# sp-uhh/audio-visual-vad

Measured on AMD Instinct MI355X. Metric: AV frame-pairs/sec (fwd+bwd), higher is better.
Workload: dtype f32; 1 GPU; AV_net fused training step (WaveNet-W0 encoder + ResNet-18 trunk + concat + 2xLSTM1024 + FC, masked BCE, backward, RCCL all-reduce, fused Adam): BASELINE configs[3]/[4] per-GPU shard; per_gpu_frame_pairs=1024, global_frame_pairs=1024, sequences_per_gpu=64, parallelism=dp1, reserved_cus=0, reported_block=median

## Files before the change

### audio-visual-vad_amd/avvad/_lib.py

```python
import ctypes as C
import os

import torch

_HERE = os.path.dirname(os.path.abspath(__file__))
LIB_PATH = os.environ.get("AVVAD_LIB") or os.path.join(os.path.dirname(_HERE), "lib", "libavvad_hip.so")

TRUNK_NCONV = 20
ABI_VERSION = 3
SCORE_CHUNK = 4096
MIX_CHUNK = 4096
SPECTRAL_CHUNK = 2048
_ERR = {-1: "AVVAD_EINVAL (bad descriptor / unsupported shape)", -2: "AVVAD_EWORKSPACE (workspace too small)",
        -3: "AVVAD_ELAUNCH (kernel launch failed)"}

FP = C.c_void_p


class AvvadError(RuntimeError):
    pass


class GemmDesc(C.Structure):
    _fields_ = [(n, C.c_int) for n in ("M", "N", "K", "lda", "ldb", "ldc", "transA", "transB", "accumulate",
# ... 36 lines not shown

class StftDesc(C.Structure):
    _fields_ = [("B", C.c_int), ("L", C.c_long), ("n_fft", C.c_int), ("hop", C.c_int), ("T", C.c_int), ("eps", C.c_float)]


class StftStreamDesc(C.Structure):
    _fields_ = [("B", C.c_int), ("L", C.c_int), ("n_fft", C.c_int), ("hop", C.c_int), ("T", C.c_int), ("M", C.c_int),
                ("eps", C.c_float), ("norm_eps", C.c_float)]


class IstftDesc(C.Structure):
    _fields_ = [(n, C.c_int) for n in ("B", "T", "n_fft", "hop", "start", "out_pitch", "mask_mode")]


class IstftStreamDesc(C.Structure):
    _fields_ = [(n, C.c_int) for n in ("B", "T", "n_fft", "hop", "L", "M", "mask_mode")]


class TargetDesc(C.Structure):
    _fields_ = [("B", C.c_int), ("L", C.c_long), ("n_fft", C.c_int), ("hop", C.c_int), ("T", C.c_int), ("center", C.c_int),
                ("eps", C.c_float), ("vad_coef", C.c_double), ("ibm_coef", C.c_double)]


class LipDesc(C.Structure):
    _fields_ = [("B", C.c_int), ("n_max", C.c_int), ("rows", C.c_long), ("T", C.c_int), ("W", C.c_int), ("H", C.c_int),
                ("p", C.c_int), ("q", C.c_int), ("quantize", C.c_int), ("norm_eps", C.c_float)]


class LstmDesc(C.Structure):
    _fields_ = [("B", C.c_int), ("T", C.c_int), ("In", C.c_int), ("H", C.c_int), ("lengths", FP),
                ("save_for_backward", C.c_int)]


SIGNATURES = {
    "avvad_version": (C.c_char_p, []),
    "avvad_abi_version": (C.c_int, []),
    "avvad_set_option": (C.c_int, [C.c_char_p, C.c_int]),
    "avvad_get_option": (C.c_int, [C.c_char_p]),
    "avvad_engine_workspace": (C.c_size_t, []),
    "avvad_gemm_f32": (C.c_int, [FP, FP, FP, FP, C.POINTER(GemmDesc), FP, C.c_size_t, FP]),
    "avvad_wavenet_workspace": (C.c_size_t, [C.POINTER(WavenetDesc)]),
    "avvad_wavenet_fwd": (C.c_int, [FP, C.POINTER(WavenetPtrs), FP, C.POINTER(WavenetDesc), FP, C.c_size_t, FP]),
    "avvad_wavenet_bwd": (C.c_int, [FP, C.POINTER(WavenetPtrs), FP, C.POINTER(WavenetPtrs), FP,
                                    C.POINTER(WavenetDesc), FP, C.c_size_t, FP]),
    "avvad_wavenet_block_fwd": (C.c_int, [FP, FP, FP, FP, FP, FP, C.c_int, C.c_int, C.c_int, FP]),
    "avvad_conv2d_pack_weights": (C.c_int, [FP, FP, FP, C.POINTER(ConvDesc), FP]),
    "avvad_conv2d_fwd": (C.c_int, [FP, FP, FP, C.POINTER(ConvDesc), FP, C.c_size_t, FP]),
    "avvad_conv2d_dgrad": (C.c_int, [FP, FP, FP, C.POINTER(ConvDesc), C.c_int, FP, C.c_size_t, FP]),
    "avvad_conv2d_wgrad": (C.c_int, [FP, FP, FP, C.POINTER(ConvDesc), FP, C.c_size_t, FP]),
    "avvad_conv2d_pack_weights_bf16": (C.c_int, [FP, FP, FP, C.POINTER(ConvDesc), FP]),
    "avvad_conv2d_fwd_bf16": (C.c_int, [FP, FP, FP, C.POINTER(ConvDesc), FP, C.c_size_t, FP]),
    "avvad_conv2d_dgrad_bf16": (C.c_int, [FP, FP, FP, C.POINTER(ConvDesc), C.c_int, FP, C.c_size_t, FP]),
    "avvad_conv2d_wgrad_bf16": (C.c_int, [FP, FP, FP, C.POINTER(ConvDesc), FP, C.c_size_t, FP]),
    "avvad_trunk_workspace": (C.c_size_t, [C.POINTER(TrunkDesc)]),
    "avvad_trunk_activation": (C.c_int, [C.POINTER(TrunkDesc), C.c_int, C.POINTER(C.c_size_t), C.POINTER(C.c_int), C.POINTER(C.c_int),
                                         C.POINTER(C.c_int)]),
    "avvad_trunk_fwd": (C.c_int, [FP, C.POINTER(TrunkParams), FP, C.POINTER(TrunkDesc), FP, C.c_size_t, FP]),
    "avvad_trunk_bwd": (C.c_int, [FP, C.POINTER(TrunkParams), FP, C.POINTER(TrunkGrads), C.POINTER(TrunkDesc), FP,
                                  C.c_size_t, FP]),
    "avvad_lstm_workspace": (C.c_size_t, [C.POINTER(LstmDesc)]),
    "avvad_lstm_layer_fwd": (C.c_int, [FP, FP, FP, FP, FP, FP, C.POINTER(LstmDesc), FP, C.c_size_t, FP]),
    "avvad_lstm_layer_bwd": (C.c_int, [FP, FP, FP, FP, FP, FP, FP, FP, FP, FP, C.POINTER(LstmDesc), FP, C.c_size_t, FP]),
    "avvad_lstm_state_workspace": (C.c_size_t, [C.POINTER(LstmDesc)]),
    "avvad_lstm_layer_fwd_state": (C.c_int, [FP] * 10 + [C.POINTER(LstmDesc), FP, C.c_size_t, FP]),
    "avvad_wavenet_stream_state_bytes": (C.c_size_t, [C.POINTER(WavenetDesc)]),
    "avvad_wavenet_stream_workspace": (C.c_size_t, [C.POINTER(WavenetDesc)]),
    "avvad_wavenet_stream_fwd": (C.c_int, [FP, C.POINTER(WavenetPtrs), FP, FP, FP, C.c_int, FP, C.c_int,
                                           C.POINTER(WavenetDesc), FP, C.c_size_t, FP]),
    "avvad_mcb_workspace": (C.c_size_t, [C.POINTER(McbDesc)]),
    "avvad_mcb_fusion_fwd": (C.c_int, [FP] * 11 + [C.POINTER(McbDesc), FP, C.c_size_t, FP]),
    "avvad_mcb_fusion_bwd": (C.c_int, [FP] * 12 + [C.POINTER(McbDesc), FP, C.c_size_t, FP]),
    "avvad_count_sketch_fwd": (C.c_int, [FP, FP, FP, FP, C.c_int, C.c_int, C.c_int, FP]),
    "avvad_count_sketch_bwd": (C.c_int, [FP, FP, FP, FP, C.c_int, C.c_int, C.c_int, FP]),
    "avvad_mcb_fwd": (C.c_int, [FP] * 7 + [C.c_int] * 4 + [FP]),
    "avvad_mcb_bwd": (C.c_int, [FP] * 9 + [C.c_int] * 4 + [FP]),
    "avvad_stft_workspace": (C.c_size_t, [C.POINTER(StftDesc)]),
    "avvad_stft": (C.c_int, [FP, FP, C.POINTER(StftDesc), C.c_int, FP, C.c_size_t, FP]),
    "avvad_stft_features": (C.c_int, [FP, FP, FP, FP, C.POINTER(StftDesc), C.c_float, FP, C.c_size_t, FP]),
    "avvad_abs_max": (C.c_int, [FP, FP, C.c_int, C.c_long, FP]),
    "avvad_stft_stream_basis_bytes": (C.c_size_t, [C.c_int]),
    "avvad_stft_stream_basis": (C.c_int, [C.c_int, FP, FP]),
    "avvad_stft_stream_fwd": (C.c_int, [FP] * 12 + [C.POINTER(StftStreamDesc), FP]),
    "avvad_stft_stream_fwd_spec": (C.c_int, [FP] * 13 + [C.POINTER(StftStreamDesc), FP]),
    "avvad_istft_stream_basis_bytes": (C.c_size_t, [C.c_int]),
    "avvad_istft_stream_basis": (C.c_int, [C.c_int, FP, FP]),
    "avvad_istft_stream_workspace": (C.c_size_t, [C.POINTER(IstftStreamDesc)]),
    "avvad_istft_stream": (C.c_int, [FP] * 10 + [C.POINTER(IstftStreamDesc), FP, C.c_size_t, FP]),
    "avvad_istft_workspace": (C.c_size_t, [C.POINTER(IstftDesc)]),
    "avvad_istft": (C.c_int, [FP, C.c_long, C.c_long, C.c_long, FP, FP, FP, FP, FP, C.POINTER(IstftDesc), FP, C.c_size_t, FP]),
    "avvad_resynth_workspace": (C.c_size_t, [C.POINTER(StftDesc), C.POINTER(IstftDesc)]),
    "avvad_resynth": (C.c_int, [FP, FP, FP, FP, FP, FP, C.POINTER(StftDesc), C.POINTER(IstftDesc), FP, C.c_size_t, FP]),
    "avvad_istft_bwd_workspace": (C.c_size_t, [C.POINTER(IstftDesc)]),
    "avvad_istft_bwd": (C.c_int, [FP, C.c_long, C.c_long, C.c_long, FP, FP, FP, FP, FP, FP, C.POINTER(IstftDesc), FP, C.c_size_t,
                                  FP]),
    "avvad_resynth_bwd_workspace": (C.c_size_t, [C.POINTER(StftDesc), C.POINTER(IstftDesc)]),
    "avvad_resynth_bwd": (C.c_int, [FP, FP, FP, FP, FP, FP, FP, C.POINTER(StftDesc), C.POINTER(IstftDesc), FP, C.c_size_t, FP]),
    "avvad_stft_complex": (C.c_int, [FP, FP, C.POINTER(StftDesc), FP, C.c_size_t, FP]),
    "avvad_stats_workspace": (C.c_size_t, [C.c_size_t, C.c_int]),
    "avvad_stats_accumulate": (C.c_int, [FP, FP, FP, C.c_int, C.c_int, C.c_int, C.c_int, FP, C.c_size_t, FP]),
    "avvad_stft_stats_workspace": (C.c_size_t, [C.POINTER(StftDesc)]),
    "avvad_stft_stats": (C.c_int, [FP, FP, FP, C.POINTER(StftDesc), FP, C.c_size_t, FP]),
    "avvad_stats_finalize": (C.c_int, [FP, C.c_int, FP, FP, FP]),
    "avvad_score_workspace": (C.c_size_t, [C.c_int, C.c_long]),
    "avvad_score_accumulate": (C.c_int, [FP, C.c_long, FP, C.c_long, FP, C.c_long, C.c_int, FP, FP, C.c_int, C.c_long, FP,
                                         C.c_size_t, FP]),
    "avvad_score_finalize": (C.c_int, [FP, C.c_int, C.c_int, FP, FP, FP]),
# ... 77 lines not shown
```

### audio-visual-vad_amd/csrc/common.h

```cpp
#pragma once
#include <hip/hip_runtime.h>
#include <stdint.h>
#include <atomic>

#include "avvad.h"

typedef float f32x16 __attribute__((ext_vector_type(16)));
typedef float f32x4 __attribute__((ext_vector_type(4)));

#include <stdio.h>
#define AVVAD_LAUNCH_CHECK()                                                                      \
  do {                                                                                            \
    hipError_t e_ = hipGetLastError();                                                            \
    if (e_ != hipSuccess) {                                                                       \
      fprintf(stderr, "avvad: HIP error '%s' after launch at %s:%d\n", hipGetErrorString(e_), __FILE__, __LINE__); \
      return AVVAD_ELAUNCH;                                                                       \
    }                                                                                             \
  } while (0)

#define AVVAD_ENTER() (void)hipGetLastError()

struct AvvadTune {
  int igemm_variant;
  int no_streamk;
  int kmajor;
  int lstm_no_fused_step;
  int lstm_no_persistent;
  int no_stem_kernel;
  int no_tall;
  int wn_no_fused_tail;
  int wn_no_tail_pair;
  int wn_no_fused_wgrad;
  int no_fixup1;
  int no_buf;
  int wn_flat;
  int wn_dx;
  int wn_grid;
  int wn_bwd_t;
  int bf16;
  int stagger;
  int cls_cap;
  int no_cls;
  int no_fused_stats;
  int no_s2_cls;
  int no_conv64;
  int bwd_max_cus;
  int max_cus;
};
AvvadTune& avvad_tune();
struct BwdCuCap {
  int saved;
  BwdCuCap() : saved(avvad_tune().max_cus) {
    const int b = avvad_tune().bwd_max_cus;
    if (b > 0 && (saved <= 0 || b < saved)) avvad_tune().max_cus = b;
  }
  ~BwdCuCap() { avvad_tune().max_cus = saved; }
};
static inline int grid_cus() {
  const int m = avvad_tune().max_cus;
  return (m > 0 && m < 256) ? m : 256;
}

template <auto Kernel>
int allow_large_lds(size_t bytes, size_t limit) {
  if (bytes <= 64 * 1024) return AVVAD_OK;
  static std::atomic<unsigned char> allowed[64];
  int dev = -1;
  if (hipGetDevice(&dev) != hipSuccess) return AVVAD_ELAUNCH;
  const bool known = dev >= 0 && dev < 64;
  if (known && allowed[dev].load(std::memory_order_acquire)) return AVVAD_OK;
  if (hipFuncSetAttribute(reinterpret_cast<const void*>(Kernel), hipFuncAttributeMaxDynamicSharedMemorySize, (int)limit) != hipSuccess)
    return AVVAD_ELAUNCH;
  if (known) allowed[dev].store(1, std::memory_order_release);
  return AVVAD_OK;
}

static inline int cdiv(long a, long b) { return (int)((a + b - 1) / b); }
static inline size_t align_up(size_t v, size_t a) { return (v + a - 1) / a * a; }
static inline bool ws_misaligned(const void* p) { return ((uintptr_t)p & 15) != 0; }
__device__ __forceinline__ int clamp_count(int v, int hi) { return v < 0 ? 0 : (v > hi ? hi : v); }

__device__ __forceinline__ f32x16 mfma32(float a, float b, f32x16 c) {
  return __builtin_amdgcn_mfma_f32_32x32x2f32(a, b, c, 0, 0, 0);
}
__device__ __forceinline__ float relu1(float x) {
  const int v = __builtin_bit_cast(int, x);
  return __builtin_bit_cast(float, v > 0 ? v : 0);
// ... 56 lines not shown
```

### audio-visual-vad_amd/csrc/misc.hip

```cpp
#include "common.h"

extern "C" const char* avvad_version(void) { return "avvad-hip 0.1 (gfx950, fp32 MFMA)"; }
extern "C" int avvad_abi_version(void) { return AVVAD_ABI_VERSION; }

#include <stdlib.h>
#include <string.h>
namespace {
struct OptName { const char* name; const char* env; int AvvadTune::*field; };
const OptName kOpts[] = {
    {"igemm_variant", "AVVAD_IGEMM_VARIANT", &AvvadTune::igemm_variant},
    {"no_streamk", "AVVAD_NO_STREAMK", &AvvadTune::no_streamk},
    {"kmajor", "AVVAD_KMAJOR", &AvvadTune::kmajor},
    {"lstm_no_fused_step", "AVVAD_LSTM_NO_FUSED_STEP", &AvvadTune::lstm_no_fused_step},
    {"lstm_no_persistent", "AVVAD_LSTM_NO_PERSISTENT", &AvvadTune::lstm_no_persistent},
    {"no_stem_kernel", "AVVAD_NO_STEM_KERNEL", &AvvadTune::no_stem_kernel},
    {"no_tall", "AVVAD_NO_TALL", &AvvadTune::no_tall},
    {"wn_no_fused_tail", "AVVAD_WN_NO_FUSED_TAIL", &AvvadTune::wn_no_fused_tail},
    {"wn_no_tail_pair", "AVVAD_WN_NO_TAIL_PAIR", &AvvadTune::wn_no_tail_pair},
    {"wn_no_fused_wgrad", "AVVAD_WN_NO_FUSED_WGRAD", &AvvadTune::wn_no_fused_wgrad},
    {"wn_bwd_t", "AVVAD_WN_BWD_T", &AvvadTune::wn_bwd_t},
    {"no_buf", "AVVAD_NO_BUF", &AvvadTune::no_buf},
    {"no_fixup1", "AVVAD_NO_FIXUP1", &AvvadTune::no_fixup1},
    {"no_conv64", "AVVAD_NO_CONV64", &AvvadTune::no_conv64},
    {"no_s2_cls", "AVVAD_NO_S2_CLS", &AvvadTune::no_s2_cls},
    {"wn_flat", "AVVAD_WN_FLAT", &AvvadTune::wn_flat},
    {"wn_grid", "AVVAD_WN_GRID", &AvvadTune::wn_grid},
    {"wn_dx", "AVVAD_WN_DX", &AvvadTune::wn_dx},
    {"bf16", "AVVAD_BF16", &AvvadTune::bf16},
    {"no_fused_stats", "AVVAD_NO_FUSED_STATS", &AvvadTune::no_fused_stats},
    {"no_cls", "AVVAD_NO_CLS", &AvvadTune::no_cls},
    {"cls_cap", "AVVAD_CLS_CAP", &AvvadTune::cls_cap},
    {"stagger", "AVVAD_STAGGER", &AvvadTune::stagger},
    {"max_cus", "AVVAD_MAX_CUS", &AvvadTune::max_cus},
    {"bwd_max_cus", "AVVAD_BWD_MAX_CUS", &AvvadTune::bwd_max_cus},
};
int parse_opt(const char* name, const char* v) {
  if (!strcmp(name, "igemm_variant")) return v[0] == 'd' ? 0 : (v[0] == 's' ? 1 : (v[0] == 'w' ? 2 : atoi(v)));
  if (!strcmp(name, "no_streamk")) return v[0] == 'a' ? 1 : (v[0] >= '0' && v[0] <= '9' && !v[1] ? 10 + (v[0] - '0') : atoi(v));
  if (!strcmp(name, "max_cus") || !strcmp(name, "bwd_max_cus") || !strcmp(name, "wn_flat") || !strcmp(name, "wn_grid") || !strcmp(name, "wn_dx") || !strcmp(name, "wn_bwd_t") || !strcmp(name, "no_fixup1") || !strcmp(name, "cls_cap")) return atoi(v);
  return (v[0] && strcmp(v, "0")) ? 1 : 0;
}
}

AvvadTune& avvad_tune() {
  static AvvadTune t = [] {
    AvvadTune x;
    memset(&x, 0, sizeof(x));
    x.igemm_variant = -1;
    for (const OptName& o : kOpts) {
      const char* v = getenv(o.env);
      if (v && v[0]) x.*(o.field) = parse_opt(o.name, v);
    }
    return x;
  }();
  return t;
}

extern "C" int avvad_set_option(const char* name, int value) {
  if (!name) return AVVAD_EINVAL;
  for (const OptName& o : kOpts)
    if (!strcmp(o.name, name)) { avvad_tune().*(o.field) = value; return AVVAD_OK; }
  return AVVAD_EINVAL;
}

extern "C" int avvad_get_option(const char* name) {
  if (!name) return AVVAD_EINVAL;
  for (const OptName& o : kOpts)
    if (!strcmp(o.name, name)) return avvad_tune().*(o.field);
  return AVVAD_EINVAL;
}

namespace {

__global__ void __launch_bounds__(1024)
    bce_masked_kernel(const float* __restrict__ logits, const float* __restrict__ targets, const int* __restrict__ lengths,
                      float* __restrict__ loss, float* __restrict__ dlogits, int B, int T, int Y, float eps) {
  __shared__ float sm[1024];
// ... 256 lines not shown
```

### audio-visual-vad_amd/csrc/trunk.hip

```cpp
#include "bgemm.h"
#include "conv64.h"

using convop::Geom;

namespace {

#include "bn_kernels.h"

constexpr int NCONV = AVVAD_TRUNK_NCONV;

constexpr int NBLOCK = 8;
constexpr int WIDTHS[4] = {64, 128, 256, 512};

struct Block {
  int stage, width;
  int h, w;
  long M;
  bool ds;
  int i1, i2, id;
  size_t in;
  size_t c1, a1;
  size_t c2, cd;
  size_t out, qm;
};
// ... 977 lines not shown
extern "C" int avvad_debug_prof_clk(unsigned long long* out, int n) {
  hipMemcpyFromSymbol(out, HIP_SYMBOL(igemm::g_prof_clk), sizeof(unsigned long long) * n);
  return 0;
}
extern "C" int avvad_debug_prof_hw(unsigned long long* out, int n) {
  hipMemcpyFromSymbol(out, HIP_SYMBOL(igemm::g_prof_hw), sizeof(unsigned long long) * n);
  return 0;
}
#endif
extern "C" int avvad_conv2d_dgrad(const float* dy, const float* wd, float* dx, const avvad_conv_desc* d, int accumulate,
                                  void* ws, size_t ws_bytes, avvad_stream_t s) {
  return conv2d_dgrad(false, dy, wd, dx, d, accumulate, ws, ws_bytes, s);
}
extern "C" int avvad_conv2d_wgrad(const float* x, const float* dy, float* dw_packed, const avvad_conv_desc* d, void* ws,
                                  size_t ws_bytes, avvad_stream_t s) {
  return conv2d_wgrad(false, x, dy, dw_packed, d, ws, ws_bytes, s);
}

namespace {
__global__ void pack_weights_bf16(const float* __restrict__ w, __bf16* __restrict__ wf16, __bf16* __restrict__ wd16, int Co, int C, int KS) {
  const int T = KS * KS, n = Co * C * T;
  for (int i = blockIdx.x * blockDim.x + threadIdx.x; i < n; i += gridDim.x * blockDim.x) {
    int r = i;
    const int tap = r % T; r /= T;
    const int c = r % C; const int co = r / C;
    const __bf16 v = (__bf16)w[i];
    wf16[(long)co * (T * C) + ((c >> 6) * T + tap) * 64 + (c & 63)] = v;
    if (wd16) wd16[(long)c * (T * Co) + ((co >> 6) * T + tap) * 64 + (co & 63)] = v;
  }
}
}
extern "C" int avvad_conv2d_pack_weights_bf16(const float* w_oihw, void* wf16, void* wd16, const avvad_conv_desc* d, avvad_stream_t s) {
  AVVAD_ENTER();
  Geom g;
  if (!w_oihw || !wf16 || !conv_geom(d, &g) || g.C % 64 || g.Co % 64) return AVVAD_EINVAL;
  hipLaunchKernelGGL(pack_weights_bf16, dim3(ew_grid((long)g.Co * g.C * g.KS * g.KS)), dim3(256), 0, (hipStream_t)s, w_oihw,
                     (__bf16*)wf16, (__bf16*)wd16, g.Co, g.C, g.KS);
  AVVAD_LAUNCH_CHECK();
  return AVVAD_OK;
}
extern "C" int avvad_conv2d_fwd_bf16(const void* x16, const void* wf16, float* y, const avvad_conv_desc* d, void* ws, size_t ws_bytes,
                                     avvad_stream_t s) {
  return conv2d_fwd(true, x16, wf16, y, d, ws, ws_bytes, s);
}
extern "C" int avvad_conv2d_dgrad_bf16(const void* dy16, const void* wd16, float* dx, const avvad_conv_desc* d, int accumulate,
                                       void* ws, size_t ws_bytes, avvad_stream_t s) {
  return conv2d_dgrad(true, dy16, wd16, dx, d, accumulate, ws, ws_bytes, s);
}
extern "C" int avvad_conv2d_wgrad_bf16(const void* x16, const void* dy16, float* dw_packed, const avvad_conv_desc* d, void* ws,
                                       size_t ws_bytes, avvad_stream_t s) {
  return conv2d_wgrad(true, x16, dy16, dw_packed, d, ws, ws_bytes, s);
}

extern "C" size_t avvad_trunk_workspace(const avvad_trunk_desc* d) {
  if (!trunk_desc_ok(d)) return 0;
  const Plan p = make_plan(d);
  return p.total * sizeof(float);
}

extern "C" int avvad_trunk_activation(const avvad_trunk_desc* d, int index, size_t* offset_floats, int* C, int* H, int* W) {
  constexpr int ARGMAX = 1 + 2 * NBLOCK;
  if (!trunk_desc_ok(d) || index < 0 || index > ARGMAX || !offset_floats || !C || !H || !W) return AVVAD_EINVAL;
  if (index == ARGMAX && !d->save_for_backward) return AVVAD_EINVAL;
  const Plan p = make_plan(d);
  if (index == 0 || index == ARGMAX) {
    *offset_floats = index == 0 ? p.p0 : p.am; *C = 64; *H = p.h[2]; *W = p.w[2];
    return AVVAD_OK;
  }
  const Block& k = p.block[(index - 1) / 2];
  *offset_floats = (index - 1) % 2 == 0 ? k.a1 : k.out;
  *C = k.width; *H = k.h; *W = k.w;
  return AVVAD_OK;
}

extern "C" int avvad_trunk_fwd(const float* frames, const avvad_trunk_params* prm, float* feat, const avvad_trunk_desc* d,
                               void* wsv, size_t ws_bytes, avvad_stream_t sv) {
  AVVAD_ENTER();
  if (!frames || !prm || !feat || !wsv || ws_misaligned(wsv) || !trunk_desc_ok(d)) return AVVAD_EINVAL;
  const Plan p = make_plan(d);
  if (ws_bytes < p.total * sizeof(float)) return AVVAD_EWORKSPACE;
  const Run r{p, (float*)wsv, prm, nullptr, d, (hipStream_t)sv};
  hipStream_t s = r.s; int rc;
  const bool b16 = native_bf16();
  const bool save = d->save_for_backward;
  PackTab tab;
  const int nb = tab_shapes(tab, p, cdiv(64 * 49, 256));
  for (int i = 0; i < NCONV; ++i) {
    tab.w[i] = prm->conv_w[i];
    tab.wf[i] = r.at(p.wf[i]);
    tab.wd[i] = (i > 0 && save) ? r.at(p.wd[i]) : nullptr;
    tab.wf16[i] = (b16 && i > 0) ? reinterpret_cast<__bf16*>(r.at(p.wf16[i])) : nullptr;
    tab.wd16[i] = (b16 && i > 0 && save) ? reinterpret_cast<__bf16*>(r.at(p.wd16[i])) : nullptr;
  }
  hipLaunchKernelGGL(pack_all, dim3(nb), dim3(256), 0, s, tab);
  if ((rc = conv_bn(r, 0, frames, r.at(p.c0)))) return rc;
  const BnSlots bn0 = r.bn(0);
  unsigned* am = save ? reinterpret_cast<unsigned*>(r.at(p.am)) : nullptr;
  auto pool = b16 ? stem_bn_relu_pool<true> : stem_bn_relu_pool<false>;
  hipLaunchKernelGGL(pool, dim3(ew_grid((long)d->N * p.h[2] * p.w[2] * 16)), dim3(256), 0, s, r.at(p.c0), bn0.scale, bn0.shift, r.at(p.p0), am,
                     d->N, p.h[1], p.w[1], p.h[2], p.w[2]);
  auto act = b16 ? bn_act<true, false> : bn_act<false, false>;
  auto act_id = b16 ? bn_act<true, true> : bn_act<false, false>;
  for (const Block& k : p.block) {
    const int C = k.width;
    const long nq = k.M * C / 4;
    const float* x = r.at(k.in);
    unsigned char* qmo = save ? reinterpret_cast<unsigned char*>(r.at(k.qm)) : nullptr;
    const BnSlots bn1 = r.bn(k.i1), bn2 = r.bn(k.i2);
    if ((rc = conv_bn(r, k.i1, x, r.at(k.c1)))) return rc;
    hipLaunchKernelGGL(act, dim3(ew_grid(nq)), dim3(256), 0, s, r.at(k.c1), bn1.scale, bn1.shift, NOF, NOF, NOF, r.at(k.a1), nq, C, 1,
                       (unsigned char*)nullptr);
    if ((rc = conv_bn(r, k.i2, r.at(k.a1), r.at(k.c2)))) return rc;
    if (k.ds) {
      if ((rc = conv_bn(r, k.id, x, r.at(k.cd)))) return rc;
      const BnSlots bnd = r.bn(k.id);
      hipLaunchKernelGGL(act, dim3(ew_grid(nq)), dim3(256), 0, s, r.at(k.c2), bn2.scale, bn2.shift, r.at(k.cd), bnd.scale, bnd.shift,
                         r.at(k.out), nq, C, 1, qmo);
    } else {
      hipLaunchKernelGGL(act_id, dim3(ew_grid(nq)), dim3(256), 0, s, r.at(k.c2), bn2.scale, bn2.shift, x, NOF, NOF, r.at(k.out), nq, C, 1, qmo);
    }
  }
  const Block& last = p.block[NBLOCK - 1];
  auto avg = b16 ? avgpool_fwd<true> : avgpool_fwd<false>;
  hipLaunchKernelGGL(avg, dim3(ew_grid((long)d->N * last.width)), dim3(256), 0, s, r.at(last.out), feat, d->N, last.h * last.w, last.width);
  AVVAD_LAUNCH_CHECK();
  return AVVAD_OK;
}

extern "C" int avvad_trunk_bwd(const float* frames, const avvad_trunk_params* prm, const float* dfeat,
                               const avvad_trunk_grads* g, const avvad_trunk_desc* d, void* wsv, size_t ws_bytes,
                               avvad_stream_t sv) {
  AVVAD_ENTER();
  BwdCuCap cu_cap;
  if (!frames || !prm || !dfeat || !g || !wsv || ws_misaligned(wsv) || !trunk_desc_ok(d) || !d->save_for_backward) return AVVAD_EINVAL;
  const Plan p = make_plan(d);
  if (ws_bytes < p.total * sizeof(float)) return AVVAD_EWORKSPACE;
  const Run r{p, (float*)wsv, prm, g, d, (hipStream_t)sv};
  hipStream_t s = r.s; int rc;
  float *G0 = r.at(p.G[0]), *G1 = r.at(p.G[1]), *G2 = r.at(p.G[2]), *G3 = r.at(p.G[3]);
  const Block& last = p.block[NBLOCK - 1];
  hipLaunchKernelGGL(avgpool_bwd, dim3(ew_grid(last.M * last.width)), dim3(256), 0, s, dfeat, G0, d->N, last.h * last.w, last.width);
  const bool b16 = native_bf16();
  const size_t* wd = b16 ? p.wd16 : p.wd;
  auto wgrad = [&](int i, const float* x, const float* dy) {
    return g->conv_w[i] ? conv_wgrad(i > 0 && b16, x, dy, r.at(p.wg[i]), p.geom[i], s, r.at(p.slab)) : AVVAD_OK;
  };
  auto dgrad = [&](int i, const float* dy, float* dx, int acc) { return conv_dgrad(b16, dy, r.at(wd[i]), dx, p.geom[i], acc, s, r.at(p.slab)); };
  for (int kb = NBLOCK - 1; kb >= 0; --kb) {
    const Block& k = p.block[kb];
    const float* x = r.at(k.in);
    BnBwd under_out, under_own;
    under_out.ymask = r.at(k.out);
    under_out.qmask = reinterpret_cast<const unsigned char*>(r.at(k.qm));
    under_out.out16 = under_own.out16 = b16; under_own.own_relu = true;
    if (k.ds) {
      if ((rc = bn_backward(r, k.i2, r.at(k.c2), G0, G1, under_out))) return rc;
      if ((rc = bn_backward(r, k.id, r.at(k.cd), G0, G2, under_out))) return rc;
      if ((rc = wgrad(k.id, x, G2))) return rc;
      if ((rc = dgrad(k.id, G2, G3, 0))) return rc;
    } else {
      under_out.gout = G3;
      if ((rc = bn_backward(r, k.i2, r.at(k.c2), G0, G1, under_out))) return rc;
    }
    if ((rc = wgrad(k.i2, r.at(k.a1), G1))) return rc;
    if ((rc = dgrad(k.i2, G1, G2, 0))) return rc;
    if ((rc = bn_backward(r, k.i1, r.at(k.c1), G2, G1, under_own))) return rc;
    if ((rc = wgrad(k.i1, x, G1))) return rc;
    if ((rc = dgrad(k.i1, G1, G3, 1))) return rc;
    float* t = G0; G0 = G3; G3 = t;
  }
  if (g->conv_w[0] || g->bn_w[0] || g->bn_b[0]) {
    float* g0 = r.at(p.g0);
    const BnSlots bn0 = r.bn(0);
    const bool fuse0 = !avvad_tune().no_fused_stats;
    int grid0 = ew_grid((long)d->N * p.h[1] * p.w[1] * 16);
    if (fuse0 && grid0 > 2048) grid0 = 2048;
    hipLaunchKernelGGL(stem_pool_relu_bwd, dim3(grid0), dim3(256), 0, s, r.at(p.c0), bn0.scale, bn0.shift,
                       reinterpret_cast<const unsigned*>(r.at(p.am)), G0, g0, d->N, p.h[1], p.w[1], p.h[2], p.w[2],
                       fuse0 ? bn0.mean : NOF, fuse0 ? bn0.invstd : NOF, fuse0 ? r.part() : (double*)nullptr);
    BnBwd stem; stem.reduced_chunks = fuse0 ? grid0 : 0;
    if ((rc = bn_backward(r, 0, r.at(p.c0), g0, g0, stem))) return rc;
    if ((rc = wgrad(0, frames, g0))) return rc;
  }
  UnpackTab tab;
  const int nb = tab_shapes(tab, p, cdiv(64 * 3 * 49, 256));
  bool any = false;
  for (int i = 0; i < NCONV; ++i) {
    tab.pk[i] = r.at(p.wg[i]);
    tab.dw[i] = g->conv_w[i];
    any = any || g->conv_w[i];
  }
  if (any) hipLaunchKernelGGL(unpack_all, dim3(nb), dim3(256), 0, s, tab);
  AVVAD_LAUNCH_CHECK();
  return AVVAD_OK;
}
```

### include/avvad.h

```cpp
#ifndef AVVAD_H
#define AVVAD_H

#include <stddef.h>
#include <stdint.h>

#ifdef __cplusplus
extern "C" {
#endif

typedef void* avvad_stream_t;

#define AVVAD_OK 0
#define AVVAD_EINVAL (-1)
#define AVVAD_EWORKSPACE (-2)
#define AVVAD_ELAUNCH (-3)

#define AVVAD_ABI_VERSION 3
const char* avvad_version(void);
int avvad_abi_version(void);

int avvad_set_option(const char* name, int value);
int avvad_get_option(const char* name);

typedef struct {
// ... 50 lines not shown
size_t avvad_wavenet_workspace(const avvad_wavenet_desc* d);
int avvad_wavenet_fwd(const float* wave, const avvad_wavenet_params* p, float* out,
                      const avvad_wavenet_desc* d, void* ws, size_t ws_bytes, avvad_stream_t s);
int avvad_wavenet_bwd(const float* wave, const avvad_wavenet_params* p, const float* dout,
                      const avvad_wavenet_grads* g, float* dwave, const avvad_wavenet_desc* d,
                      void* ws, size_t ws_bytes, avvad_stream_t s);

int avvad_wavenet_block_fwd(const float* s_in, const float* w_dil, const float* b_dil, const float* w_dense,
                            const float* b_dense, float* s_out, int B, int Lin, int dil, avvad_stream_t s);

#define AVVAD_TRUNK_NCONV 20

typedef struct {
  int N, H, W;
  int training;
  float momentum;
  float eps;
  int save_for_backward;
} avvad_trunk_desc;

typedef struct {
  const float* conv_w[AVVAD_TRUNK_NCONV];
  const float* bn_w[AVVAD_TRUNK_NCONV];
  const float* bn_b[AVVAD_TRUNK_NCONV];
  float* bn_rm[AVVAD_TRUNK_NCONV];
  float* bn_rv[AVVAD_TRUNK_NCONV];
} avvad_trunk_params;

typedef struct {
  float* conv_w[AVVAD_TRUNK_NCONV];
  float* bn_w[AVVAD_TRUNK_NCONV];
  float* bn_b[AVVAD_TRUNK_NCONV];
} avvad_trunk_grads;

typedef struct {
  int N, H, W, C, Co, KS, stride, pad;
} avvad_conv_desc;
int avvad_conv2d_pack_weights(const float* w_oihw, float* wf, float* wd, const avvad_conv_desc* d,
                              avvad_stream_t s);
int avvad_conv2d_fwd(const float* x, const float* wf, float* y, const avvad_conv_desc* d, void* ws,
                     size_t ws_bytes, avvad_stream_t s);
int avvad_conv2d_dgrad(const float* dy, const float* wd, float* dx, const avvad_conv_desc* d,
                       int accumulate, void* ws, size_t ws_bytes, avvad_stream_t s);
int avvad_conv2d_wgrad(const float* x, const float* dy, float* dw_packed, const avvad_conv_desc* d, void* ws,
                       size_t ws_bytes, avvad_stream_t s);

int avvad_conv2d_pack_weights_bf16(const float* w_oihw, void* wf16, void* wd16, const avvad_conv_desc* d, avvad_stream_t s);
int avvad_conv2d_fwd_bf16(const void* x16, const void* wf16, float* y, const avvad_conv_desc* d, void* ws, size_t ws_bytes,
                          avvad_stream_t s);
int avvad_conv2d_dgrad_bf16(const void* dy16, const void* wd16, float* dx, const avvad_conv_desc* d, int accumulate,
                            void* ws, size_t ws_bytes, avvad_stream_t s);
int avvad_conv2d_wgrad_bf16(const void* x16, const void* dy16, float* dw_packed, const avvad_conv_desc* d, void* ws,
                            size_t ws_bytes, avvad_stream_t s);

size_t avvad_trunk_workspace(const avvad_trunk_desc* d);
int avvad_trunk_activation(const avvad_trunk_desc* d, int index, size_t* offset_floats, int* C, int* H, int* W);
int avvad_trunk_fwd(const float* frames, const avvad_trunk_params* p, float* feat ,
                    const avvad_trunk_desc* d, void* ws, size_t ws_bytes, avvad_stream_t s);
int avvad_trunk_bwd(const float* frames, const avvad_trunk_params* p, const float* dfeat,
                    const avvad_trunk_grads* g, const avvad_trunk_desc* d, void* ws, size_t ws_bytes,
                    avvad_stream_t s);

typedef struct {
  int B, T, In, H;
  const int* lengths;
  int save_for_backward;
} avvad_lstm_desc;
size_t avvad_lstm_workspace(const avvad_lstm_desc* d);
int avvad_lstm_layer_fwd(const float* x, const float* w_ih, const float* w_hh, const float* b_ih,
                         const float* b_hh, float* y, const avvad_lstm_desc* d, void* ws,
                         size_t ws_bytes, avvad_stream_t s);
int avvad_lstm_layer_bwd(const float* x, const float* w_ih, const float* w_hh, const float* y,
                         const float* dy, float* dx, float* dw_ih, float* dw_hh, float* db_ih,
                         float* db_hh, const avvad_lstm_desc* d, void* ws, size_t ws_bytes,
                         avvad_stream_t s);

size_t avvad_lstm_state_workspace(const avvad_lstm_desc* d);
int avvad_lstm_layer_fwd_state(const float* x, const float* w_ih, const float* w_hh, const float* b_ih,
                               const float* b_hh, const float* h0, const float* c0, float* y, float* hT, float* cT,
                               const avvad_lstm_desc* d, void* ws, size_t ws_bytes, avvad_stream_t s);

size_t avvad_wavenet_stream_state_bytes(const avvad_wavenet_desc* d);
size_t avvad_wavenet_stream_workspace(const avvad_wavenet_desc* d);
int avvad_wavenet_stream_fwd(const float* chunk, const avvad_wavenet_params* p, float* state, const int* n_valid,
                             const int* skip, int k, float* out, int out_frames, const avvad_wavenet_desc* d, void* ws,
                             size_t ws_bytes, avvad_stream_t s);

typedef struct {
  int rows, A, V, D;
  float eps;
  int training;
  float momentum;
  int save_for_backward;
} avvad_mcb_desc;
size_t avvad_mcb_workspace(const avvad_mcb_desc* d);
int avvad_mcb_fusion_fwd(const float* audio, const float* video, const int64_t* h1, const float* s1,
                         const int64_t* h2, const float* s2, const float* bn_w, const float* bn_b,
                         float* bn_rm, float* bn_rv, float* out, const avvad_mcb_desc* d, void* ws,
                         size_t ws_bytes, avvad_stream_t s);
int avvad_mcb_fusion_bwd(const float* audio, const float* video, const int64_t* h1, const float* s1,
                         const int64_t* h2, const float* s2, const float* bn_w, const float* dout,
                         float* daudio, float* dvideo, float* dbn_w, float* dbn_b,
                         const avvad_mcb_desc* d, void* ws, size_t ws_bytes, avvad_stream_t s);

int avvad_count_sketch_fwd(const float* x, const int64_t* h, const float* s, float* out, int rows, int In, int D,
                           avvad_stream_t st);
// ... 186 lines not shown
```

Baseline: 60860 frame-pairs/s.

## Fuse stride-2 downsample block dgrad with shortcut 1x1 dgrad via parity-decomposed kernel

Adds a specialised data-gradient kernel for the 64->128 stride-2 3x3 conv in the ResNet trunk. It splits the input-gradient pixels into four parity classes and computes each from only the taps that reach it. The shortcut 1x1 stride-2 conv dgrad is folded into the same accumulation, replacing two dgrad launches plus an accumulate pass. A standalone pointwise stride-2 dgrad kernel is also added for other downsample shortcuts; it writes zeros to the pixels the stride skips. Both kernels reuse the stream-K-style split/fixup planning of the existing implicit GEMM. They are limited to f32 and to specific shapes, and fall back to the generic path otherwise.

```diff
diff --git a/audio-visual-vad_amd/avvad/_lib.py b/audio-visual-vad_amd/avvad/_lib.py
--- a/audio-visual-vad_amd/avvad/_lib.py
+++ b/audio-visual-vad_amd/avvad/_lib.py
@@ -112,6 +112,8 @@
     "avvad_conv2d_fwd_bf16": (C.c_int, [FP, FP, FP, C.POINTER(ConvDesc), FP, C.c_size_t, FP]),
     "avvad_conv2d_dgrad_bf16": (C.c_int, [FP, FP, FP, C.POINTER(ConvDesc), C.c_int, FP, C.c_size_t, FP]),
     "avvad_conv2d_wgrad_bf16": (C.c_int, [FP, FP, FP, C.POINTER(ConvDesc), FP, C.c_size_t, FP]),
+    "avvad_entry_dgrad": (C.c_int, [FP, FP, FP, FP, FP, C.POINTER(ConvDesc), FP, C.c_size_t, FP]),
+    "avvad_pointwise_dgrad": (C.c_int, [FP, FP, FP, C.POINTER(ConvDesc), FP, C.c_size_t, FP]),
     "avvad_trunk_workspace": (C.c_size_t, [C.POINTER(TrunkDesc)]),
     "avvad_trunk_activation": (C.c_int, [C.POINTER(TrunkDesc), C.c_int, C.POINTER(C.c_size_t), C.POINTER(C.c_int), C.POINTER(C.c_int),
                                          C.POINTER(C.c_int)]),
diff --git a/audio-visual-vad_amd/csrc/common.h b/audio-visual-vad_amd/csrc/common.h
--- a/audio-visual-vad_amd/csrc/common.h
+++ b/audio-visual-vad_amd/csrc/common.h
@@ -33,6 +33,7 @@
   int wn_no_fused_wgrad;
   int no_fixup1;
   int no_buf;
+  int no_entry;
   int wn_flat;
   int wn_dx;
   int wn_grid;
diff --git a/audio-visual-vad_amd/csrc/entry.h b/audio-visual-vad_amd/csrc/entry.h
--- /dev/null
+++ b/audio-visual-vad_amd/csrc/entry.h
@@ -0,0 +1,282 @@
+#pragma once
+#include "common.h"
+
+namespace entry {
+
+constexpr int NW = 8;
+constexpr int MAXROWS = 512;
+
+struct Prod { int G, base, rt; };
+struct Sched { int w1, w2, w3, w4; int has_ds; Prod ds, c0, c1, c2, c3; };
+
+struct Cut {
+  unsigned R, G, it0, g, nb;
+  bool split;
+  __device__ __forceinline__ void init(int te, const Prod& P, int kt) {
+    split = P.rt > 0 && te >= P.base;
+    if (!split) return;
+    R = (unsigned)P.rt * (unsigned)kt; G = (unsigned)P.G; it0 = (unsigned)(te - P.base) * (unsigned)kt;
+    g = ((it0 + 1u) * G + R - 1u) / R - 1u;
+    nb = (g + 1u) * R / G;
+  }
+  __device__ __forceinline__ bool ends(int j, int kt) {
+    if (j == kt - 1) return true;
+    if (!split || it0 + (unsigned)j + 1u < nb) return false;
+    do { ++g; nb = (g + 1u) * R / G; } while (nb <= it0 + (unsigned)j + 1u);
+    return true;
+  }
+};
+
+#define ENTRY_CONTRACT(av, row0)                                                                                  \
+  do {                                                                                                            \
+    const float* const bt_ = wl + ((row0) + lh) * 64 + li;                                                        \
+    float b_[2][8];                                                                                               \
+    _Pragma("unroll") for (int s_ = 0; s_ < 4; ++s_) { b_[0][2 * s_] = bt_[s_ * 128]; b_[0][2 * s_ + 1] = bt_[s_ * 128 + 32]; } \
+    _Pragma("unroll") for (int j_ = 0; j_ < 4; ++j_) {                                                            \
+      if (j_ < 3) {                                                                                               \
+        _Pragma("unroll") for (int s_ = 0; s_ < 4; ++s_) {                                                        \
+          b_[(j_ + 1) & 1][2 * s_] = bt_[((j_ + 1) * 4 + s_) * 128];                                              \
+          b_[(j_ + 1) & 1][2 * s_ + 1] = bt_[((j_ + 1) * 4 + s_) * 128 + 32];                                     \
+        }                                                                                                         \
+      }                                                                                                           \
+      __builtin_amdgcn_sched_barrier(0);                                                                          \
+      _Pragma("unroll") for (int s_ = 0; s_ < 4; ++s_) {                                                          \
+        const int i_ = j_ * 4 + s_;                                                                               \
+        const float a_ = lh ? av[i_ >> 1][2 * (i_ & 1) + 1] : av[i_ >> 1][2 * (i_ & 1)];                          \
+        acc0 = mfma32(a_, b_[j_ & 1][2 * s_], acc0);                                                              \
+        acc1 = mfma32(a_, b_[j_ & 1][2 * s_ + 1], acc1);                                                          \
+      }                                                                                                           \
+      __builtin_amdgcn_sched_barrier(0);                                                                          \
+    }                                                                                                             \
+  } while (0)
+#define ENTRY_FLUSH(last)                                                                                         \
+  do {                                                                                                            \
+    if (npiece == 0) {                                                                                            \
+      _Pragma("unroll") for (int r_ = 0; r_ < 16; ++r_) { val0[r_] = val0[r_] + (acc0[r_] + 0.f); val1[r_] = val1[r_] + (acc1[r_] + 0.f); } \
+    } else {                                                                                                      \
+      _Pragma("unroll") for (int r_ = 0; r_ < 16; ++r_) { sum0[r_] = sum0[r_] + acc0[r_]; sum1[r_] = sum1[r_] + acc1[r_]; } \
+    }                                                                                                             \
+    ++npiece;                                                                                                     \
+    _Pragma("unroll") for (int r_ = 0; r_ < 16; ++r_) { acc0[r_] = 0.f; acc1[r_] = 0.f; }                         \
+    if (last) {                                                                                                   \
+      if (npiece > 1) {                                                                                           \
+        _Pragma("unroll") for (int r_ = 0; r_ < 16; ++r_) { val0[r_] = val0[r_] + sum0[r_]; val1[r_] = val1[r_] + sum1[r_]; } \
+      }                                                                                                           \
+      _Pragma("unroll") for (int r_ = 0; r_ < 16; ++r_) { sum0[r_] = 0.f; sum1[r_] = 0.f; }                       \
+      npiece = 0;                                                                                                 \
+    }                                                                                                             \
+  } while (0)
+
+__global__ void __launch_bounds__(NW * 64, 2)
+    dgrad_kernel(const float* __restrict__ dy, const float* __restrict__ wd, const float* __restrict__ dd, const float* __restrict__ wdd,
+                 float* __restrict__ dx, const int N, const int H, const int W, const int Ho, const int Wo, const Sched sc) {
+  __shared__ __attribute__((aligned(16))) float wl[MAXROWS * 64];
+  const int t = threadIdx.x, lane = t & 63, wave = t >> 6;
+  const int li = lane & 31, lh = lane >> 5;
+  const int bid = blockIdx.x;
+  const int q = (bid >= sc.w1 ? 1 : 0) + (bid >= sc.w2 ? 1 : 0) + (bid >= sc.w3 ? 1 : 0);
+  const int ph = q >> 1, pw = q & 1;
+  const int b0 = q == 0 ? 0 : (q == 1 ? sc.w1 : (q == 2 ? sc.w2 : sc.w3));
+  const int b1 = q == 0 ? sc.w1 : (q == 1 ? sc.w2 : (q == 2 ? sc.w3 : sc.w4));
+  const Prod pc = q == 0 ? sc.c0 : (q == 1 ? sc.c1 : (q == 2 ? sc.c2 : sc.c3));
+  const int Hc = (H - ph + 1) >> 1, Wc = (W - pw + 1) >> 1, HWc = Hc * Wc, Mc = N * HWc;
+  const unsigned mg_hw = HWc > 1 ? (unsigned)(0x100000000ull / (unsigned)HWc + 1ull) : 0u;
+  const unsigned mg_w = Wc > 1 ? (unsigned)(0x100000000ull / (unsigned)Wc + 1ull) : 0u;
+  const int ntap = (1 + ph) * (1 + pw), tsh = ph + pw;
+  const int nds = (q == 0 && sc.has_ds) ? 4 : 0;
+  const int ktc = 4 * ntap, nstep = nds + ktc;
+  const __amdgpu_buffer_rsrc_t rx = brsrc2g(dy);
+  const __amdgpu_buffer_rsrc_t rd = brsrc2g(sc.has_ds ? dd : dy);
+  const __amdgpu_buffer_rsrc_t ro = brsrc2g(dx);
+  const long T = ((long)Mc + 31) / 32, G = b1 - b0;
+  const long t_lo = (bid - b0) * T / G, t_hi = (bid - b0 + 1) * T / G;
+
+  struct Step { int delta, need, row; bool ds; };
+  auto step = [&](int s) -> Step {
+    if (s < nds) return {s * 128, 0, ntap * 128 + s * 32, true};
+    const int j = s - nds, cc = j >> tsh, tp = j & (ntap - 1);
+    const int ia = pw ? tp >> 1 : tp, ib = pw ? tp & 1 : 0;
+    const int dho = ph ? 1 - ia : 0, dwo = pw ? 1 - ib : 0;
+    return {(dho * Wo + dwo) * 512 + cc * 128, dho | (dwo << 1), tp * 128 + cc * 32, false};
+  };
+  int pixbase = 0, vmask = 0;
+  auto tile_ctx = [&](long tile) {
+    const int m = (int)tile * 32 + li;
+    const int n = mg_hw ? (int)__umulhi((unsigned)m, mg_hw) : m, r = m - n * HWc;
+    const int hc = mg_w ? (int)__umulhi((unsigned)r, mg_w) : r, wc = r - hc * Wc;
+    const int okh = hc + 1 < Ho ? 1 : 0, okw = wc + 1 < Wo ? 1 : 0;
+    vmask = m < Mc ? (1 | (okh << 1) | (okw << 2) | ((okh & okw) << 3)) : 0;
+    pixbase = ((n * Ho + hc) * Wo + wc) * 512;
+  };
+  f4v a0[8], a1[8];
+  f32x16 acc0, acc1, val0, val1, sum0, sum1;
+  auto fetch = [&](f4v (&av)[8], int s) {
+    const Step st = step(s);
+    const int vo = ((vmask >> st.need) & 1) ? pixbase + st.delta : BUF_OOB;
+    if (st.ds) {
+#pragma unroll
+      for (int j = 0; j < 8; ++j) av[j] = bload4(rd, vo + j * 16, 0);
+    } else {
+#pragma unroll
+      for (int j = 0; j < 8; ++j) av[j] = bload4(rx, vo + j * 16, 0);
+    }
+  };
+
+  long tile = t_lo + wave;
+  if (tile < t_hi) {
+    tile_ctx(tile);
+    fetch(a0, 0);
+  }
+  for (int u = 0; u < ntap + (nds ? 1 : 0); ++u) {
+    const int ia = pw ? u >> 1 : u, ib = pw ? u & 1 : 0;
+    const int kh = ph ? 2 * ia : 1, kw = pw ? 2 * ib : 1;
+    const float4* src = reinterpret_cast<const float4*>(u < ntap ? wd + (long)(kh * 3 + kw) * 128 * 64 : wdd);
+    float4* dst = reinterpret_cast<float4*>(wl + u * 128 * 64);
+#pragma unroll
+    for (int i = t; i < 128 * 16; i += NW * 64) dst[i] = src[i];
+  }
+  __syncthreads();
+#pragma unroll
+  for (int r = 0; r < 16; ++r) { acc0[r] = 0.f; acc1[r] = 0.f; sum0[r] = 0.f; sum1[r] = 0.f; }
+  for (; tile < t_hi; tile += NW) {
+#pragma unroll
+    for (int r = 0; r < 16; ++r) { val0[r] = 0.f; val1[r] = 0.f; }
+    const int m0 = (int)tile * 32;
+    const int te = __builtin_amdgcn_readfirstlane(m0 >> 7);
+    Cut cutd, cutc;
+    cutd.split = false;
+    if (nds) cutd.init(te, sc.ds, 4);
+    cutc.init(te, pc, ktc);
+    int npiece = 0;
+    const bool more = tile + NW < t_hi;
+#pragma unroll 1
+    for (int s = 0; s < nstep; s += 2) {
+      fetch(a1, s + 1);
+      ENTRY_CONTRACT(a0, step(s).row);
+      if (s < nds ? cutd.ends(s, 4) : cutc.ends(s - nds, ktc)) ENTRY_FLUSH(s == nds - 1 || s == nstep - 1);
+      if (s + 2 < nstep) {
+        fetch(a0, s + 2);
+      } else if (more) {
+        tile_ctx(tile + NW);
+        fetch(a0, 0);
+      }
+      ENTRY_CONTRACT(a1, step(s + 1).row);
+      if (s + 1 < nds ? cutd.ends(s + 1, 4) : cutc.ends(s + 1 - nds, ktc)) ENTRY_FLUSH(s + 1 == nds - 1 || s + 1 == nstep - 1);
+    }
+#pragma unroll
+    for (int r = 0; r < 16; ++r) {
+      const int m = m0 + mfma32_row(r, lh);
+      const int n = mg_hw ? (int)__umulhi((unsigned)m, mg_hw) : m, rr = m - n * HWc;
+      const int hc = mg_w ? (int)__umulhi((unsigned)rr, mg_w) : rr, wc = rr - hc * Wc;
+      const int vo = m < Mc ? (((n * H + 2 * hc + ph) * W + 2 * wc + pw) * 64 + li) * 4 : BUF_OOB;
+      bstore(val0[r], ro, vo, 0);
+      bstore(val1[r], ro, vo, 128);
+    }
+  }
+}
+
+__global__ void __launch_bounds__(NW * 64, 2)
+    pw_dgrad_kernel(const float* __restrict__ dd, const float* __restrict__ wd, float* __restrict__ dx, const int N, const int H,
+                    const int W, const int Ho, const int Wo, const int C, const int Co, const int ncb, const int bn, const int ntn,
+                    const Prod pp) {
+  __shared__ __attribute__((aligned(16))) float wl[MAXROWS * 64];
+  const int t = threadIdx.x, lane = t & 63, wave = t >> 6;
+  const int li = lane & 31, lh = lane >> 5;
+  const int pg = blockIdx.x / ncb, cb = blockIdx.x - pg * ncb;
+  const int HWo = Ho * Wo, M = N * HWo;
+  const unsigned mg_hw = HWo > 1 ? (unsigned)(0x100000000ull / (unsigned)HWo + 1ull) : 0u;
+  const unsigned mg_w = Wo > 1 ? (unsigned)(0x100000000ull / (unsigned)Wo + 1ull) : 0u;
+  const int kt = Co >> 5;
+  const __amdgpu_buffer_rsrc_t rx = brsrc2g(dd);
+  const __amdgpu_buffer_rsrc_t ro = brsrc2g(dx);
+  const long T = ((long)M + 31) / 32, G = gridDim.x / ncb;
+  const long t_lo = pg * T / G, t_hi = (pg + 1) * T / G;
+  const int pix = Co * 4;
+  f4v a0[8], a1[8];
+  f32x16 acc0, acc1, val0, val1, sum0, sum1;
+  auto fetch = [&](f4v (&av)[8], long tile, int s) {
+    const int m = (int)tile * 32 + li;
+    const int vo = m < M ? m * pix + s * 128 : BUF_OOB;
+#pragma unroll
+    for (int j = 0; j < 8; ++j) av[j] = bload4(rx, vo + j * 16, 0);
+  };
+  long tile = t_lo + wave;
+  if (tile < t_hi) fetch(a0, tile, 0);
+  for (int i = t; i < Co * 16; i += NW * 64)
+    reinterpret_cast<float4*>(wl)[i] = *reinterpret_cast<const float4*>(wd + (long)(i >> 4) * C + cb * 64 + (i & 15) * 4);
+  __syncthreads();
+#pragma unroll
+  for (int r = 0; r < 16; ++r) { acc0[r] = 0.f; acc1[r] = 0.f; sum0[r] = 0.f; sum1[r] = 0.f; }
+  for (; tile < t_hi; tile += NW) {
+#pragma unroll
+    for (int r = 0; r < 16; ++r) { val0[r] = 0.f; val1[r] = 0.f; }
+    const int m0 = (int)tile * 32;
+    const int te = __builtin_amdgcn_readfirstlane((m0 >> 7) * ntn + cb * 64 / bn);
+    Cut cut;
+    cut.init(te, pp, kt);
+    int npiece = 0;
+    const bool more = tile + NW < t_hi;
+#pragma unroll 1
+    for (int s = 0; s < kt; s += 2) {
+      fetch(a1, tile, s + 1);
+      ENTRY_CONTRACT(a0, s * 32);
+      if (cut.ends(s, kt)) ENTRY_FLUSH(false);
+      if (s + 2 < kt) fetch(a0, tile, s + 2);
+      else if (more) fetch(a0, tile + NW, 0);
+      ENTRY_CONTRACT(a1, (s + 1) * 32);
+      if (cut.ends(s + 1, kt)) ENTRY_FLUSH(s + 1 == kt - 1);
+    }
+#pragma unroll
+    for (int r = 0; r < 16; ++r) {
+      const int m = m0 + mfma32_row(r, lh);
+      const int n = mg_hw ? (int)__umulhi((unsigned)m, mg_hw) : m, rr = m - n * HWo;
+      const int ho = mg_w ? (int)__umulhi((unsigned)rr, mg_w) : rr, wo = rr - ho * Wo;
+      const bool in = m < M, right = 2 * wo + 1 < W, below = 2 * ho + 1 < H;
+      const int vo = (((n * H + 2 * ho) * W + 2 * wo) * C + cb * 64 + li) * 4;
+      const int v00 = in ? vo : BUF_OOB, v01 = in && right ? vo + C * 4 : BUF_OOB;
+      const int v10 = in && below ? vo + W * C * 4 : BUF_OOB, v11 = in && below && right ? vo + (W + 1) * C * 4 : BUF_OOB;
+      bstore(val0[r], ro, v00, 0);
+      bstore(val1[r], ro, v00, 128);
+      bstore(0.f, ro, v01, 0); bstore(0.f, ro, v01, 128);
+      bstore(0.f, ro, v10, 0); bstore(0.f, ro, v10, 128);
+      bstore(0.f, ro, v11, 0); bstore(0.f, ro, v11, 128);
+    }
+  }
+}
+#undef ENTRY_CONTRACT
+#undef ENTRY_FLUSH
+
+static inline int pw_grid(long M, int ncb, int cus) {
+  const long T = (M + 31) / 32;
+  long gp = cus / ncb > 0 ? cus / ncb : 1;
+  if (gp > T) gp = T;
+  return (int)gp * ncb;
+}
+
+static inline int plan(int N, int H, int W, bool has_ds, int cus, Sched* sc) {
+  long tiles[4], work[4];
+  int g[4], total = 0;
+  long all = 0;
+  for (int q = 0; q < 4; ++q) {
+    const int ph = q >> 1, pw = q & 1;
+    const long Mc = (long)N * ((H - ph + 1) / 2) * ((W - pw + 1) / 2);
+    tiles[q] = (Mc + 31) / 32;
+    work[q] = tiles[q] * (2 * (1 + ph) * (1 + pw) + (q == 0 && has_ds ? 2 : 0));
+    g[q] = tiles[q] > 0 ? 1 : 0;
+    total += g[q];
+    all += tiles[q];
+  }
+  const long want = all < cus ? all : cus;
+  while (total < want) {
+    int best = -1;
+    for (int q = 0; q < 4; ++q)
+      if (g[q] > 0 && g[q] < tiles[q] && (best < 0 || work[q] * g[best] > work[best] * g[q])) best = q;
+    if (best < 0) break;
+    ++g[best]; ++total;
+  }
+  sc->w1 = g[0]; sc->w2 = sc->w1 + g[1]; sc->w3 = sc->w2 + g[2]; sc->w4 = sc->w3 + g[3];
+  sc->has_ds = has_ds ? 1 : 0;
+  return total;
+}
+
+}
diff --git a/audio-visual-vad_amd/csrc/misc.hip b/audio-visual-vad_amd/csrc/misc.hip
--- a/audio-visual-vad_amd/csrc/misc.hip
+++ b/audio-visual-vad_amd/csrc/misc.hip
@@ -23,6 +23,7 @@
     {"no_fixup1", "AVVAD_NO_FIXUP1", &AvvadTune::no_fixup1},
     {"no_conv64", "AVVAD_NO_CONV64", &AvvadTune::no_conv64},
     {"no_s2_cls", "AVVAD_NO_S2_CLS", &AvvadTune::no_s2_cls},
+    {"no_entry", "AVVAD_NO_ENTRY", &AvvadTune::no_entry},
     {"wn_flat", "AVVAD_WN_FLAT", &AvvadTune::wn_flat},
     {"wn_grid", "AVVAD_WN_GRID", &AvvadTune::wn_grid},
     {"wn_dx", "AVVAD_WN_DX", &AvvadTune::wn_dx},
diff --git a/audio-visual-vad_amd/csrc/trunk.hip b/audio-visual-vad_amd/csrc/trunk.hip
--- a/audio-visual-vad_amd/csrc/trunk.hip
+++ b/audio-visual-vad_amd/csrc/trunk.hip
@@ -1053,6 +1053,90 @@
   return conv2d_wgrad(true, x16, dy16, dw_packed, d, ws, ws_bytes, s);
 }
 
+#include "entry.h"
+static inline bool entry_dgrad_ok(const Geom& g, bool b16) {
+  const long HWc = (long)((g.H + 1) / 2) * ((g.W + 1) / 2);
+  return !b16 && avvad_tune().bf16 == 0 && !avvad_tune().no_entry && g.C == 64 && g.Co == 128 && g.KS == 3 && g.stride == 2 &&
+         g.pad == 1 && fits_buf((long)g.N * g.H * g.W * 64) && fits_buf((long)g.N * g.Ho * g.Wo * 128) &&
+         (unsigned long)(g.N * HWc + 64) * (unsigned long)HWc < 0x100000000ull;
+}
+static inline bool entry_sibling(const Geom& g, const Geom& gd) {
+  return gd.KS == 1 && gd.stride == 2 && gd.pad == 0 && gd.N == g.N && gd.H == g.H && gd.W == g.W && gd.C == g.C && gd.Co == g.Co &&
+         gd.Ho == g.Ho && gd.Wo == g.Wo;
+}
+static bool entry_prod(long M, int ktiles, int bn, int ncols, bool slab, entry::Prod* p) {
+  const AvvadTune& tn = avvad_tune();
+  if (tn.igemm_variant >= 0) return false;
+  *p = entry::Prod{1, 0, 0};
+  const long ntiles = (long)cdiv(M, 128L) * cdiv(ncols, bn);
+  if (ntiles <= 0) return true;
+  const igemm::Rounds r = igemm::plan_rounds(ntiles, ktiles, igemm::workers(bn == 128 ? 2 : 4, 128, bn), slab, 1);
+  const int depth = tn.no_fixup1 == 1 ? 0 : (tn.no_fixup1 > 1 ? tn.no_fixup1 : igemm::FIXUP1_DEPTH);
+  if (r.rem > 0 && (r.G + r.rem - 1) / r.rem > depth) return false;
+  *p = entry::Prod{(int)r.G, (int)(r.full_rounds * r.G), r.rem};
+  return true;
+}
+static bool entry_dgrad_plan(const Geom& g, bool has_ds, bool slab, entry::Sched* sc, int* grid) {
+  *grid = entry::plan(g.N, g.H, g.W, has_ds, grid_cus(), sc);
+  entry::Prod* const pc[4] = {&sc->c0, &sc->c1, &sc->c2, &sc->c3};
+  for (int q = 0; q < 4; ++q) {
+    const int ph = q >> 1, pw = q & 1;
+    if (!entry_prod((long)g.N * ((g.H - ph + 1) / 2) * ((g.W - pw + 1) / 2), 4 * (1 + ph) * (1 + pw), 64, 64, slab, pc[q])) return false;
+  }
+  return entry_prod((long)g.N * ((g.H + 1) / 2) * ((g.W + 1) / 2), 4, 64, 64, slab, &sc->ds);
+}
+static int entry_dgrad_launch(const float* dy, const float* wd, const float* dd, const float* wdd, float* dx, const Geom& g, hipStream_t s,
+                              const entry::Sched& sc, int grid) {
+  hipLaunchKernelGGL(entry::dgrad_kernel, dim3(grid), dim3(entry::NW * 64), 0, s, dy, wd, dd, wdd, dx, g.N, g.H, g.W, g.Ho, g.Wo, sc);
+  AVVAD_LAUNCH_CHECK();
+  return AVVAD_OK;
+}
+static inline bool pw_dgrad_ok(const Geom& g, bool b16) {
+  const long HWo = (long)g.Ho * g.Wo;
+  return !b16 && avvad_tune().bf16 == 0 && !avvad_tune().no_entry && g.KS == 1 && g.stride == 2 && g.pad == 0 && g.C % 64 == 0 &&
+         g.Co % 128 == 0 && g.Co <= entry::MAXROWS && fits_buf((long)g.N * g.H * g.W * g.C) && fits_buf(g.N * HWo * g.Co) &&
+         (unsigned long)(g.N * HWo + 64) * (unsigned long)HWo < 0x100000000ull;
+}
+static bool pw_dgrad_plan(const Geom& g, bool slab, entry::Prod* pp) {
+  return entry_prod((long)g.N * g.Ho * g.Wo, g.Co / 32, g.C <= 64 ? 64 : 128, g.C, slab, pp);
+}
+static int pw_dgrad_launch(const float* dd, const float* wd, float* dx, const Geom& g, hipStream_t s, const entry::Prod& pp) {
+  const int ncb = g.C / 64, bn = g.C <= 64 ? 64 : 128;
+  const int grid = entry::pw_grid((long)g.N * g.Ho * g.Wo, ncb, grid_cus());
+  hipLaunchKernelGGL(entry::pw_dgrad_kernel, dim3(grid), dim3(entry::NW * 64), 0, s, dd, wd, dx, g.N, g.H, g.W, g.Ho, g.Wo, g.C, g.Co, ncb, bn,
+                     cdiv(g.C, bn), pp);
+  AVVAD_LAUNCH_CHECK();
+  return AVVAD_OK;
+}
+extern "C" int avvad_pointwise_dgrad(const float* dd, const float* wd, float* dx, const avvad_conv_desc* d, void* ws, size_t ws_bytes,
+                                     avvad_stream_t s) {
+  AVVAD_ENTER();
+  Geom g;
+  if (!dd || !wd || !dx || !conv_geom(d, &g) || ws_misaligned(ws)) return AVVAD_EINVAL;
+  float* slab = slab_of(ws, ws_bytes);
+  entry::Prod pp;
+  if (pw_dgrad_ok(g, false) && pw_dgrad_plan(g, slab != nullptr, &pp)) return pw_dgrad_launch(dd, wd, dx, g, (hipStream_t)s, pp);
+  return conv_dgrad(false, dd, wd, dx, g, 0, (hipStream_t)s, slab);
+}
+extern "C" int avvad_entry_dgrad(const float* dy, const float* wd, const float* dd, const float* wdd, float* dx, const avvad_conv_desc* d,
+                                 void* ws, size_t ws_bytes, avvad_stream_t s) {
+  AVVAD_ENTER();
+  Geom g;
+  if (!dy || !wd || !dx || (dd == nullptr) != (wdd == nullptr) || !conv_geom(d, &g) || ws_misaligned(ws)) return AVVAD_EINVAL;
+  Geom gd = g;
+  gd.KS = 1; gd.pad = 0;
+  gd.Ho = (g.H - 1) / g.stride + 1; gd.Wo = (g.W - 1) / g.stride + 1;
+  if (dd && (gd.Ho != g.Ho || gd.Wo != g.Wo)) return AVVAD_EINVAL;
+  float* slab = slab_of(ws, ws_bytes);
+  entry::Sched sc;
+  int grid;
+  if (entry_dgrad_ok(g, false) && (!dd || entry_sibling(g, gd)) && entry_dgrad_plan(g, dd != nullptr, slab != nullptr, &sc, &grid))
+    return entry_dgrad_launch(dy, wd, dd, wdd, dx, g, (hipStream_t)s, sc, grid);
+  if (dd)
+    if (const int rc = conv_dgrad(false, dd, wdd, dx, gd, 0, (hipStream_t)s, slab)) return rc;
+  return conv_dgrad(false, dy, wd, dx, g, dd ? 1 : 0, (hipStream_t)s, slab);
+}
+
 extern "C" size_t avvad_trunk_workspace(const avvad_trunk_desc* d) {
   if (!trunk_desc_ok(d)) return 0;
   const Plan p = make_plan(d);
@@ -1154,20 +1238,32 @@
     under_out.ymask = r.at(k.out);
     under_out.qmask = reinterpret_cast<const unsigned char*>(r.at(k.qm));
     under_out.out16 = under_own.out16 = b16; under_own.own_relu = true;
+    entry::Sched esc;
+    entry::Prod epp;
+    int egrid = 0;
+    const bool own_entry = k.ds && entry_dgrad_ok(p.geom[k.i1], b16) && entry_sibling(p.geom[k.i1], p.geom[k.id]) &&
+                           entry_dgrad_plan(p.geom[k.i1], true, true, &esc, &egrid);
     if (k.ds) {
       if ((rc = bn_backward(r, k.i2, r.at(k.c2), G0, G1, under_out))) return rc;
       if ((rc = bn_backward(r, k.id, r.at(k.cd), G0, G2, under_out))) return rc;
       if ((rc = wgrad(k.id, x, G2))) return rc;
-      if ((rc = dgrad(k.id, G2, G3, 0))) return rc;
+      if (!own_entry) {
+        rc = pw_dgrad_ok(p.geom[k.id], b16) && pw_dgrad_plan(p.geom[k.id], true, &epp) ? pw_dgrad_launch(G2, r.at(wd[k.id]), G3, p.geom[k.id], s, epp)
+                                                                                     : dgrad(k.id, G2, G3, 0);
+        if (rc) return rc;
+      }
     } else {
       under_out.gout = G3;
       if ((rc = bn_backward(r, k.i2, r.at(k.c2), G0, G1, under_out))) return rc;
     }
     if ((rc = wgrad(k.i2, r.at(k.a1), G1))) return rc;
-    if ((rc = dgrad(k.i2, G1, G2, 0))) return rc;
-    if ((rc = bn_backward(r, k.i1, r.at(k.c1), G2, G1, under_own))) return rc;
+    float* const Ga = own_entry ? G0 : G2;
+    if ((rc = dgrad(k.i2, G1, Ga, 0))) return rc;
+    if ((rc = bn_backward(r, k.i1, r.at(k.c1), Ga, G1, under_own))) return rc;
     if ((rc = wgrad(k.i1, x, G1))) return rc;
-    if ((rc = dgrad(k.i1, G1, G3, 1))) return rc;
+    if (own_entry) {
+      if ((rc = entry_dgrad_launch(G1, r.at(wd[k.i1]), G2, r.at(wd[k.id]), G3, p.geom[k.i1], s, esc, egrid))) return rc;
+    } else if ((rc = dgrad(k.i1, G1, G3, 1))) return rc;
     float* t = G0; G0 = G3; G3 = t;
   }
   if (g->conv_w[0] || g->bn_w[0] || g->bn_b[0]) {
diff --git a/include/avvad.h b/include/avvad.h
--- a/include/avvad.h
+++ b/include/avvad.h
@@ -126,6 +126,12 @@
                             void* ws, size_t ws_bytes, avvad_stream_t s);
 int avvad_conv2d_wgrad_bf16(const void* x16, const void* dy16, float* dw_packed, const avvad_conv_desc* d, void* ws,
                             size_t ws_bytes, avvad_stream_t s);
+
+int avvad_entry_dgrad(const float* dy, const float* wd, const float* dd, const float* wdd, float* dx,
+                      const avvad_conv_desc* d, void* ws, size_t ws_bytes, avvad_stream_t s);
+
+int avvad_pointwise_dgrad(const float* dd, const float* wd, float* dx, const avvad_conv_desc* d, void* ws,
+                          size_t ws_bytes, avvad_stream_t s);
 
 size_t avvad_trunk_workspace(const avvad_trunk_desc* d);
 int avvad_trunk_activation(const avvad_trunk_desc* d, int index, size_t* offset_floats, int* C, int* H, int* W);
```

Measured after the change: 61230 frame-pairs/s, median of 6. No clear change (+0.6%).
